# PoeBlu/open-network-insight

Hardware: AMD Instinct MI355X
Metric: netflow records scored/sec (whole node) + Gibbs iters/sec, 20-topic LDA (higher is better)
Workload: dtype fp32

## Files before the change

### csrc/kernels/corpus.hip

```cpp
#include <hipcub/hipcub.hpp>

#include "oni_common.h"

namespace {

constexpr int kB = 256;
inline unsigned nblk(int64_t n) { return (unsigned)((n + kB - 1) / kB > 0 ? (n + kB - 1) / kB : 1); }

struct Arena {
  char* base;
  size_t used = 0;
  template <class T>
  T* take(size_t n) {
    used = (used + 255) & ~size_t(255);
    T* p = base ? reinterpret_cast<T*>(base + used) : nullptr;
    used += n * sizeof(T);
    return p;
  }
};

__global__ void k_iota(int32_t* __restrict__ v, int64_t n) {
  const int64_t i = (int64_t)blockIdx.x * kB + threadIdx.x;
  if (i < n) v[i] = (int32_t)i;
}
// ... 139 lines not shown
  const int64_t i = (int64_t)blockIdx.x * kB + threadIdx.x;
  if (i >= n_chunks) return;
  int64_t lo = 0, hi = D;
  while (hi - lo > 1) {
    const int64_t mid = (lo + hi) >> 1;
    if (chunk_first[mid] <= i) lo = mid; else hi = mid;
  }
  const int64_t c = i - chunk_first[lo];
  const int64_t nt = tok_ptr[lo + 1] - tok_ptr[lo];
  const int64_t p0 = c * L;
  const int64_t ln = nt - p0 < L ? nt - p0 : L;
  cdoc[i] = (int32_t)lo;
  cpos0[i] = (int32_t)p0;
  clen[i] = (int32_t)ln;
  cmulti[i] = (chunk_first[lo + 1] - chunk_first[lo]) > 1 ? 1 : 0;
  key[i] = (uint32_t)(L - ln);
}

__global__ void k_chunk_gather(const int32_t* __restrict__ order, int64_t n_chunks, int64_t n_pad_total,
                               const int32_t* __restrict__ cdoc, const int32_t* __restrict__ cpos0,
                               const int32_t* __restrict__ clen, const uint8_t* __restrict__ cmulti,
                               const int32_t* __restrict__ doc_keys, int32_t* __restrict__ o_doc,
                               int32_t* __restrict__ o_pos0, int32_t* __restrict__ o_len, uint8_t* __restrict__ o_multi,
                               int32_t* __restrict__ o_key) {
  const int64_t i = (int64_t)blockIdx.x * kB + threadIdx.x;
  if (i >= n_pad_total) return;
  if (i < n_chunks) {
    const int32_t s = order[i];
    const int32_t d = cdoc[s];
    o_doc[i] = d;
    o_pos0[i] = cpos0[s];
    o_len[i] = clen[s];
    o_multi[i] = cmulti[s];
    o_key[i] = doc_keys[d];
  } else {
    o_doc[i] = -1;
    o_pos0[i] = 0;
    o_len[i] = 0;
    o_multi[i] = 0;
    o_key[i] = 0;
  }
}

__global__ void k_slice_len(const int32_t* __restrict__ o_len, int64_t ns, int S, int32_t* __restrict__ slice_len,
                            int64_t* __restrict__ slice_w) {
  const int64_t s = (int64_t)blockIdx.x * kB + threadIdx.x;
  if (s < ns) {
    slice_len[s] = o_len[s * S];
    slice_w[s] = (int64_t)o_len[s * S] * S;
  }
  if (s == ns) slice_w[ns] = 0;
}

__global__ void k_word_keys(const uint32_t* __restrict__ tok_word, int64_t n, uint32_t V, uint32_t* __restrict__ key) {
  const int64_t i = (int64_t)blockIdx.x * kB + threadIdx.x;
  if (i < n) {
    const uint32_t w = tok_word[i];
    key[i] = w == oni::kPadWord ? V : w;
  }
}

__global__ void k_word_index(const uint32_t* __restrict__ ks, const int32_t* __restrict__ slot, int64_t T, int tile,
                             int32_t* __restrict__ wpos, int32_t* __restrict__ tile_wlo,
                             int32_t* __restrict__ tile_whi) {
  const int64_t i = (int64_t)blockIdx.x * kB + threadIdx.x;
  if (i >= T) return;
  wpos[slot[i]] = (int32_t)i;
  if (i % tile == 0) {
    const int64_t t = i / tile;
    const int64_t e = i + tile - 1 < T - 1 ? i + tile - 1 : T - 1;
    tile_wlo[t] = (int32_t)ks[i];
    tile_whi[t] = (int32_t)ks[e];
  }
}

__global__ void k_fill_i32(int32_t* __restrict__ p, int64_t n, int32_t v) {
  const int64_t i = (int64_t)blockIdx.x * kB + threadIdx.x;
  if (i < n) p[i] = v;
}

#define ONI_TRY(x)                          \
  do {                                       \
    const hipError_t e_ = (x);               \
    if (e_ != hipSuccess) return (int)e_;    \
  } while (0)

int bits_for(uint64_t maxv) {
  int b = 1;
  while (b < 64 && (maxv >> b)) ++b;
  return b;
}

hipError_t window_pass(void* tmp, size_t& bytes, const int32_t* perm, int32_t* keys_out, const int32_t* val,
                       int32_t* val_out, int64_t n, hipStream_t s) {
  const int pbits = bits_for(n > 1 ? (uint64_t)(n - 1) : 1);
  const int lo = pbits > 8 ? pbits - 8 : 0;
  return hipcub::DeviceRadixSort::SortPairs(tmp, bytes, reinterpret_cast<const uint32_t*>(perm),
                                            reinterpret_cast<uint32_t*>(keys_out), val, val_out, (int)n, lo, pbits,
                                            s);
}

__global__ void k_scatter(const int32_t* __restrict__ dst, const int32_t* __restrict__ val, int64_t n,
                          int32_t* __restrict__ out) {
  const unsigned per = gridDim.x / 8u;
  const unsigned t = (blockIdx.x % 8u) * per + blockIdx.x / 8u;
  const int64_t i = (int64_t)t * kB + threadIdx.x;
  if (i < n) out[dst[i]] = val[i];
}

inline unsigned nblk8(int64_t n) { return (nblk(n) + 7u) & ~7u; }

}

template <class K>
static int dict_encode_impl(const uint64_t* keys, int64_t n, int key_bits, uint64_t* uniq, int32_t* ids,
                            int64_t* n_uniq, const int32_t* weight, int64_t* counts, void* tmp, size_t* tmp_bytes,
                            hipStream_t s) {
  constexpr bool kNarrow = sizeof(K) == 4;
  Arena ar{static_cast<char*>(tmp)};
  K* kin = kNarrow ? ar.take<K>(n) : nullptr;
  K* ks = ar.take<K>(n);
// ... 281 lines not shown
    return 0;
  }
  if (nnz > 0) k_doc_pair_ptr<<<nblk(nnz), kB, 0, s>>>(pair_doc, nnz, D, doc_pair_ptr);
  else k_fill_i32<<<1, kB, 0, s>>>(reinterpret_cast<int32_t*>(doc_pair_ptr), 2 * (D + 1), 0);
  k_i32_to_i64<<<nblk(nnz + 1), kB, 0, s>>>(pair_cnt, nnz, c64);
  ONI_TRY(hipcub::DeviceScan::ExclusiveSum(cub, cbytes, c64, glob, (int)(nnz + 1), s));
  k_doc_tok<<<nblk(D + 1), kB, 0, s>>>(doc_pair_ptr, glob, D, L, doc_tok_ptr, nch, is_long);
  k_pair_tokoff<<<nblk(nnz), kB, 0, s>>>(pair_doc, glob, doc_tok_ptr, nnz, pair_tokoff);
  ONI_TRY(hipcub::DeviceScan::ExclusiveSum(cub, cbytes, nch, chunk_first, (int)(D + 1), s));
  k_iota<<<nblk(D), kB, 0, s>>>(iota, D);
  if (D > 0) ONI_TRY(hipcub::DeviceSelect::Flagged(cub, cbytes, iota, is_long, long_rows, n_long, (int)D, s));
  else ONI_TRY(hipMemsetAsync(n_long, 0, sizeof(int32_t), s));
  k_scalars3<<<1, 64, 0, s>>>(glob + nnz, chunk_first + D, n_long, scalars);
  return (int)hipGetLastError();
}

ONI_API int oni_chunk_layout(const int64_t* chunk_first, const int64_t* doc_tok_ptr, const int32_t* doc_keys,
                             int64_t D, int64_t n_chunks, int L, int S, int32_t* chunk_doc, int32_t* chunk_pos0,
                             int32_t* chunk_len, uint8_t* chunk_multi, int32_t* chunk_key, int32_t* slice_len,
                             int64_t* slice_off, void* tmp, size_t* tmp_bytes, hipStream_t s) {
  const int64_t ns = (n_chunks + S - 1) / S;
  Arena ar{static_cast<char*>(tmp)};
  int32_t* cdoc = ar.take<int32_t>(n_chunks);
  int32_t* cpos0 = ar.take<int32_t>(n_chunks);
  int32_t* clen = ar.take<int32_t>(n_chunks);
  uint8_t* cmul = ar.take<uint8_t>(n_chunks);
  uint32_t* key = ar.take<uint32_t>(n_chunks);
  uint32_t* ks = ar.take<uint32_t>(n_chunks);
  int32_t* iota = ar.take<int32_t>(n_chunks);
  int32_t* order = ar.take<int32_t>(n_chunks);
  int64_t* sw = ar.take<int64_t>(ns + 1);
  const int kbits = bits_for((uint64_t)L);
  size_t b1 = 0, b2 = 0;
  ONI_TRY(hipcub::DeviceRadixSort::SortPairs(nullptr, b1, key, ks, iota, order, (int)n_chunks, 0, kbits, s));
  ONI_TRY(hipcub::DeviceScan::ExclusiveSum(nullptr, b2, sw, slice_off, (int)(ns + 1), s));
  void* cub = ar.take<char>(b1 > b2 ? b1 : b2);
  if (!tmp) {
    *tmp_bytes = ar.used + 256;
    return 0;
  }
  size_t cbytes = b1 > b2 ? b1 : b2;
  if (n_chunks > 0) {
    k_chunks<<<nblk(n_chunks), kB, 0, s>>>(chunk_first, doc_tok_ptr, D, n_chunks, L, cdoc, cpos0, clen, cmul, key);
    k_iota<<<nblk(n_chunks), kB, 0, s>>>(iota, n_chunks);
    ONI_TRY(hipcub::DeviceRadixSort::SortPairs(cub, cbytes, key, ks, iota, order, (int)n_chunks, 0, kbits, s));
  }
  k_chunk_gather<<<nblk(ns * S), kB, 0, s>>>(order, n_chunks, ns * S, cdoc, cpos0, clen, cmul, doc_keys, chunk_doc,
                                            chunk_pos0, chunk_len, chunk_multi, chunk_key);
  k_slice_len<<<nblk(ns + 1), kB, 0, s>>>(chunk_len, ns, S, slice_len, sw);
  ONI_TRY(hipcub::DeviceScan::ExclusiveSum(cub, cbytes, sw, slice_off, (int)(ns + 1), s));
  return (int)hipGetLastError();
}

ONI_API int oni_word_index(const uint32_t* tok_word, int64_t slots, int64_t T, int64_t V, int tile,
                           int32_t* wsorted, int32_t* wslot, int32_t* wpos, int32_t* tile_wlo, int32_t* tile_whi,
                           void* tmp, size_t* tmp_bytes, hipStream_t s) {
  if (slots >= (int64_t)1 << 31) return (int)hipErrorInvalidValue;
  Arena ar{static_cast<char*>(tmp)};
  uint32_t* key = ar.take<uint32_t>(slots);
  uint32_t* ks = reinterpret_cast<uint32_t*>(wsorted);
  int32_t* iota = ar.take<int32_t>(slots);
  int32_t* slot = wslot;
  const int kbits = bits_for((uint64_t)V);
  size_t b1 = 0;
  ONI_TRY(hipcub::DeviceRadixSort::SortPairs(nullptr, b1, key, ks, iota, slot, (int)slots, 0, kbits, s));
  void* cub = ar.take<char>(b1);
  if (!tmp) {
    *tmp_bytes = ar.used + 256;
    return 0;
  }
  k_fill_i32<<<nblk(slots), kB, 0, s>>>(wpos, slots, -1);
  if (slots == 0) return (int)hipGetLastError();
  k_word_keys<<<nblk(slots), kB, 0, s>>>(tok_word, slots, (uint32_t)V, key);
  k_iota<<<nblk(slots), kB, 0, s>>>(iota, slots);
  ONI_TRY(hipcub::DeviceRadixSort::SortPairs(cub, b1, key, ks, iota, slot, (int)slots, 0, kbits, s));
  if (T > 0) k_word_index<<<nblk(T), kB, 0, s>>>(ks, slot, T, tile, wpos, tile_wlo, tile_whi);
  return (int)hipGetLastError();
}
```

### csrc/kernels/glue.hip

```cpp
#include "oni_common.h"

namespace {

__global__ __launch_bounds__(256) void k_widen_pair(const uint32_t* __restrict__ a, const uint32_t* __restrict__ b,
                                                    int64_t n, uint64_t* __restrict__ out) {
  const int64_t stride = (int64_t)gridDim.x * blockDim.x;
  for (int64_t i = (int64_t)blockIdx.x * blockDim.x + threadIdx.x; i < n; i += stride) {
    out[i] = (uint64_t)a[i];
    out[n + i] = (uint64_t)b[i];
  }
}

}

ONI_API int oni_widen_pair(const uint32_t* a, const uint32_t* b, int64_t n, uint64_t* out, hipStream_t s) {
  if (n <= 0) return 0;
  k_widen_pair<<<oni::grid_for(n, 256, 8192), 256, 0, s>>>(a, b, n, out);
  return (int)hipGetLastError();
}
```

### csrc/kernels/sell.hip

```cpp
#include "oni_common.h"

namespace {

__device__ __forceinline__ int64_t find_pair(const int64_t* __restrict__ tokoff, int64_t lo, int64_t hi, int64_t pos) {
  while (hi - lo > 1) {
    const int64_t mid = (lo + hi) >> 1;
    if (tokoff[mid] <= pos) lo = mid; else hi = mid;
  }
  return lo;
}

__global__ void k_sell_fill(const int32_t* __restrict__ chunk_doc, const int32_t* __restrict__ chunk_pos0,
                            const int32_t* __restrict__ chunk_len, int64_t n_chunks, int S,
                            const int64_t* __restrict__ slice_off, const int64_t* __restrict__ doc_pair_ptr,
                            const int64_t* __restrict__ pair_tokoff, const int32_t* __restrict__ pair_word,
                            const int32_t* __restrict__ pair_cnt, uint32_t* __restrict__ tok_word) {
  const int64_t i = (int64_t)blockIdx.x * blockDim.x + threadIdx.x;
  if (i >= n_chunks) return;
  const int d = chunk_doc[i];
  if (d < 0) return;
  const int64_t slice = i / S, lane = i % S;
  const int64_t off = slice_off[slice] + lane;
  const int64_t pos0 = chunk_pos0[i];
  const int len = chunk_len[i];
  int64_t j = find_pair(pair_tokoff, doc_pair_ptr[d], doc_pair_ptr[d + 1], pos0);
  int64_t end = pair_tokoff[j] + pair_cnt[j];
  uint32_t w = (uint32_t)pair_word[j];
  for (int s = 0; s < len; ++s) {
    const int64_t pos = pos0 + s;
    while (end <= pos) {
      ++j;
      end = pair_tokoff[j] + pair_cnt[j];
      w = (uint32_t)pair_word[j];
    }
    tok_word[off + (int64_t)s * S] = w;
  }
}

__global__ void k_sell_perm_z(const int32_t* __restrict__ chunk_doc, const int32_t* __restrict__ chunk_pos0,
                              const int32_t* __restrict__ chunk_len, int64_t n_chunks, int S,
                              const int64_t* __restrict__ slice_off, const int64_t* __restrict__ doc_tok_ptr,
                              uint8_t* __restrict__ tok_z, uint8_t* __restrict__ canon_z, int dir) {
  const int64_t i = (int64_t)blockIdx.x * blockDim.x + threadIdx.x;
  if (i >= n_chunks) return;
  const int d = chunk_doc[i];
  if (d < 0) return;
  const int64_t slice = i / S, lane = i % S;
  const int64_t off = slice_off[slice] + lane;
  const int64_t base = doc_tok_ptr[d] + chunk_pos0[i];
  const int len = chunk_len[i];
  for (int s = 0; s < len; ++s) {
    if (dir == 0) canon_z[base + s] = tok_z[off + (int64_t)s * S];
    else tok_z[off + (int64_t)s * S] = canon_z[base + s];
  }
}

}

ONI_API int oni_sell_fill(const int32_t* chunk_doc, const int32_t* chunk_pos0, const int32_t* chunk_len,
                          int64_t n_chunks, int S, const int64_t* slice_off, const int64_t* doc_pair_ptr,
                          const int64_t* pair_tokoff, const int32_t* pair_word, const int32_t* pair_cnt,
                          uint32_t* tok_word, hipStream_t s) {
  const unsigned grid = (unsigned)((n_chunks + 255) / 256);
  if (grid == 0) return 0;
  k_sell_fill<<<grid, 256, 0, s>>>(chunk_doc, chunk_pos0, chunk_len, n_chunks, S, slice_off, doc_pair_ptr,
                                   pair_tokoff, pair_word, pair_cnt, tok_word);
  return (int)hipGetLastError();
}

ONI_API int oni_sell_perm_z(const int32_t* chunk_doc, const int32_t* chunk_pos0, const int32_t* chunk_len,
                            int64_t n_chunks, int S, const int64_t* slice_off, const int64_t* doc_tok_ptr,
                            uint8_t* tok_z, uint8_t* canon_z, int dir, hipStream_t s) {
  const unsigned grid = (unsigned)((n_chunks + 255) / 256);
  if (grid == 0) return 0;
  k_sell_perm_z<<<grid, 256, 0, s>>>(chunk_doc, chunk_pos0, chunk_len, n_chunks, S, slice_off, doc_tok_ptr, tok_z,
                                     canon_z, dir);
  return (int)hipGetLastError();
}
```

### oni355/ops/__init__.py

```python
from __future__ import annotations

import os

import ctypes as C
import enum
from typing import NamedTuple

import numpy as np
import torch

from ..ref import spec
from . import _lib

__all__ = [
    "f32_keys", "i64_keys", "quantile_cuts", "bin_keys", "flow_keys", "flow_wordify", "sell_fill",
    "sell_perm_z", "gibbs_pass", "foldin_pass", "prior_rows", "theta_rows_prior", "table_lookup", "gibbs_which", "GibbsKernel", "gibbs_apply", "mh_tables", "SAMPLER_MH", "CountMode", "copy_rows", "score", "select_below", "choose_tiling",
]


def _is_dev(t: torch.Tensor) -> bool:
    return t.device.type == "cuda"


def _u32np(t: torch.Tensor) -> np.ndarray:
# ... 520 lines not shown
              wsum: torch.Tensor | None = None, wcdf: torch.Tensor | None = None) -> None:
    cdf = wcdf is not None
    if cdf == (walias is not None) or (walias is not None and wsum is None):
        raise ValueError("one word proposal table: walias + wsum, or wcdf")
    if cdf and (wcdf.shape != (q.shape[0], spec.MH_CDF_BUCKETS) or wcdf.dtype != torch.float32):
        raise ValueError("wcdf must be a [V, 16] float32 table")
    if not _is_dev(q):
        wt, ws, da, gg = spec.mh_tables(q.numpy(), nk.numpy(), ndk_src.numpy(), long_rows.numpy(), K, alpha, vbeta,
                                        word="cdf" if cdf else "alias")
        if cdf:
            wcdf.copy_(torch.from_numpy(wt))
        else:
            walias.copy_(torch.from_numpy(wt.view(np.int32)))
            wsum.copy_(torch.from_numpy(ws))
        if da.shape[0]:
            dalias.copy_(torch.from_numpy(da.view(np.int32)))
        g.copy_(torch.from_numpy(gg))
        return
    V, KS = q.shape
    p = lambda t: _lib.ptr(t) if t is not None else None
    _lib.check(_lib.lib().oni_mh_tables(_lib.ptr(q), V, K, KS, _lib.ptr(ndk_src), _lib.ptr(long_rows),
                                        long_rows.numel(), float(alpha), p(walias), p(wsum), p(wcdf),
                                        _lib.ptr(dalias), _lib.ptr(nk), float(vbeta), _lib.ptr(g), _lib.stream()),
               "oni_mh_tables")


def delta_recount(wslot, tile_wlo, tile_whi, chg_mask, tok_word, tok_z, tok_zprev, dnwk_out, KS: int, G: int) -> None:
    T = wslot.numel()
    if T == 0:
        return
    if not _is_dev(tok_z):
        sl = wslot.long()
        zn, zo = tok_z[sl].long(), tok_zprev[sl].long()
        ch = zn != zo
        w = tok_word[sl][ch].long()
        one = torch.ones(int(ch.sum()), dtype=torch.int32)
        dnwk_out.view(-1).index_add_(0, w * KS + zn[ch], one)
        dnwk_out.view(-1).index_add_(0, w * KS + zo[ch], -one)
        tok_zprev[sl[ch]] = tok_z[sl[ch]]
        return
    S = 64 // G
    wmax = max(1, RECOUNT_CELLS // KS)
    _lib.check(_lib.lib().oni_delta_recount(*map(_lib.ptr, (wslot, tile_wlo, tile_whi, chg_mask, tok_word, tok_z,
                                                            tok_zprev)), T, _lib.ptr(dnwk_out), KS,
                                            S.bit_length() - 1, G, RECOUNT_TILE, wmax, _lib.stream()),
               "oni_delta_recount")


WBITS_BLOCK = 8192


def wdelta_records(wsorted: torch.Tensor) -> torch.Tensor:
    T = wsorted.numel()
    out = torch.zeros((max(T, 1), 2), dtype=torch.int16, device=wsorted.device)
    if T:
        nb = -(-T // WBITS_BLOCK)
        w = torch.nn.functional.pad(wsorted.to(torch.int32), (0, nb * WBITS_BLOCK - T)).view(nb, WBITS_BLOCK)
        rel = (w - w[:, :1]).view(-1)[:T].clamp_(max=0xFFFF)
        out[:T, 1] = torch.where(rel >= 0x8000, rel - 0x10000, rel).to(torch.int16)
    return out.view(torch.int32).view(-1)


def wdelta_recount(wbits, wsorted, zz_w, dnwk_out, KS: int) -> None:
    T = wsorted.numel()
    if T == 0:
        return
    if not _is_dev(wsorted):
        b = wbits.numpy().view(np.uint32)
        pos = np.nonzero(np.unpackbits(b.view(np.uint8), bitorder="little")[:T])[0]
        pt = torch.from_numpy(pos)
        w = wsorted[pt].long()
        one = torch.ones(pos.size, dtype=torch.int32)
        zz = zz_w[pt].to(torch.int64) & 0xFFFF
        dnwk_out.view(-1).index_add_(0, w * KS + (zz >> 8), one)
        dnwk_out.view(-1).index_add_(0, w * KS + (zz & 0xFF), -one)
        wbits.zero_()
        return
    if zz_w.dtype != torch.int32 or zz_w.numel() < T:
        raise ValueError("zz_w must be the int32 [T] record array of wdelta_records")
    wmax = max(1, RECOUNT_CELLS // KS)
    _lib.check(_lib.lib().oni_wdelta_recount(*map(_lib.ptr, (wbits, wsorted, zz_w)), T, _lib.ptr(dnwk_out), KS,
                                             wmax, _lib.stream()), "oni_wdelta_recount")


RECOUNT_TILE = 4096
DN_AUX = 4
RECOUNT_CELLS = 2048


def exact_guard(ndk: torch.Tensor, rows: torch.Tensor, K: int, limit: int, flag: torch.Tensor) -> None:
    KS = ndk.shape[-1]
    if not _is_dev(ndk):
        ok = not bool((ndk[rows.long(), :K] > limit).any()) if rows.numel() else True
        flag.fill_(1 if ok else 0)
        return
    _lib.check(_lib.lib().oni_exact_guard(_lib.ptr(ndk), _lib.ptr(rows), int(rows.numel()), KS, K, int(limit),
                                          _lib.ptr(flag), _lib.stream()), "oni_exact_guard")


def recount(wsorted, wslot, tok_z, nwk_out, KS: int) -> None:
    T = wsorted.numel()
    if T == 0:
        return
    if not _is_dev(tok_z):
        z = (tok_z[wslot.long()] if wslot is not None else tok_z[:T]).long()
        nwk_out.view(-1).index_add_(0, wsorted.long() * KS + z, torch.ones_like(z, dtype=torch.int32))
# ... 333 lines not shown
```

### oni355/ops/_lib.py

```python
from __future__ import annotations

import ctypes as C
import os
import threading

import torch

_HERE = os.path.dirname(os.path.abspath(__file__))
LIB_DIR = os.path.join(os.path.dirname(_HERE), "_lib")
HIP_LIB_PATH = os.path.join(LIB_DIR, "liboni_hip.so")

_lock = threading.Lock()
_lib = None

vp, i32, i64, f32, u32 = C.c_void_p, C.c_int32, C.c_int64, C.c_float, C.c_uint32


class OniGibbs(C.Structure):

    _fields_ = [
        ("tok_word", vp), ("tok_z", vp), ("slice_off", vp), ("slice_len", vp),
        ("chunk_doc", vp), ("chunk_pos0", vp), ("chunk_key", vp), ("chunk_multi", vp),
        ("ndk_src", vp), ("ndk_dst", vp), ("q", vp), ("qfix", vp), ("dnwk", vp), ("dnk", vp), ("sweep_ctr", vp), ("chg_mask", vp),
        ("wpos", vp), ("z_w", vp), ("zz_w", vp), ("chg_count", vp), ("exact_guard", vp), ("tok_zlag", vp),
        ("n_slices", i64), ("K", i32), ("KS", i32), ("alpha", f32), ("seed0", u32), ("seed1", u32),
        ("nk_rep", i32), ("flags", i32),
    ]


class OniMH(C.Structure):

    _fields_ = [
        ("g", OniGibbs), ("walias", vp), ("wsum", vp), ("wcdf", vp), ("dalias", vp), ("mh_g", vp), ("chunk_dslot", vp),
        ("chunk_len", vp), ("kalpha", f32), ("inv_alpha", f32), ("lmax", i32), ("doc_moves", i32), ("wp", i32),
    ]


class OniFoldin(C.Structure):

    _fields_ = [
        ("tok_word", vp), ("tok_z", vp), ("slice_off", vp), ("slice_len", vp),
        ("chunk_doc", vp), ("chunk_pos0", vp), ("chunk_key", vp), ("chunk_multi", vp),
        ("ndk_src", vp), ("ndk_dst", vp), ("phi", vp), ("ndk_sum", vp),
        ("n_slices", i64), ("K", i32), ("KS", i32), ("alpha", f32), ("seed0", u32), ("seed1", u32),
        ("sweep_lo", i32), ("n_sweeps", i32), ("avg_from", i32), ("select", i32),
        ("prior", vp),
    ]


_REGISTRY: dict[str, list] = {
    "oni_radix_hist": [vp, i64, C.c_int, C.c_int, vp, C.c_int, u32, vp, vp],
    "oni_f32_keys": [vp, i64, vp, vp],
    "oni_i64_keys": [vp, i64, vp, vp],
    "oni_bin_keys": [vp, i64, vp, C.c_int, vp, vp],
    "oni_flow_keys": [vp, vp, vp, vp, vp, i64, vp, vp, vp, vp],
    "oni_flow_wordify": [vp, vp, vp, vp, vp, i64, vp, C.c_int, C.c_int, C.c_int, vp, vp, vp],
    "oni_sell_fill": [vp, vp, vp, i64, C.c_int, vp, vp, vp, vp, vp, vp, vp],
    "oni_sell_perm_z": [vp, vp, vp, i64, C.c_int, vp, vp, vp, vp, C.c_int, vp],
    "oni_gibbs_launch": [C.POINTER(OniGibbs), C.c_int, C.c_int, C.c_int, C.c_int, C.c_int, vp],
    "oni_gibbs_which": [C.POINTER(OniGibbs), C.c_int, C.c_int, C.c_int, C.c_int, C.c_int, C.POINTER(C.c_int),
                        C.POINTER(C.c_int)],
    "oni_gibbs_sizeof_args": [],
    "oni_exact_guard": [vp, vp, i64, C.c_int, C.c_int, C.c_int32, vp, vp],
    "oni_gibbs_mh_launch": [C.POINTER(OniMH), C.c_int, C.c_int, vp],
    "oni_mh_sizeof_args": [],
    "oni_mh_tables": [vp, i64, C.c_int, C.c_int, vp, vp, i64, f32, vp, vp, vp, vp, vp, f32, vp, vp],
    "oni_widen_pair": [vp, vp, i64, vp, vp],
    "oni_quantile_pick": [vp, vp, C.c_int, C.c_int, C.c_int, vp, vp, vp],
    "oni_tail_grid": [],
    "oni_tail_sums": [vp, vp, vp, vp, i64, i64, C.c_int, C.c_int, C.c_double, C.c_double, C.c_double, C.c_double,
                      vp, vp, vp],
    "oni_theta_rows": [vp, i64, C.c_int, C.c_int, f32, f32, vp, C.c_int, vp],
    "oni_theta_rows_prior": [vp, vp, i64, C.c_int, C.c_int, f32, vp, C.c_int, vp],
    "oni_prior_rows": [vp, vp, vp, i64, vp, i64, C.c_int, C.c_int, f32, f32, vp, vp],
    "oni_phi_rows": [vp, vp, i64, C.c_int, C.c_int, f32, f32, vp, C.c_int, C.c_int, vp],
    "oni_gibbs_apply": [vp, vp, vp, vp, vp, vp, vp, i64, C.c_int, C.c_int, f32, f32, vp, C.c_int, C.c_int, C.c_int,
                        vp, vp, vp, i64, vp, vp, vp, C.c_int, vp, i64, C.c_int, vp],
    "oni_recount": [vp, vp, vp, i64, vp, C.c_int, C.c_int, C.c_int, vp],
    "oni_recount_stream": [vp, vp, i64, vp, C.c_int, C.c_int, C.c_int, vp],
    "oni_delta_recount": [vp, vp, vp, vp, vp, vp, vp, i64, vp, C.c_int, C.c_int, C.c_int, C.c_int, C.c_int, vp],
    "oni_copy_rows": [vp, vp, vp, i64, C.c_int, vp],
    "oni_x01_pack": [vp, vp, i64, vp, i64, vp, i64, C.c_int, i64, i64, C.c_int, C.c_int, vp, vp],
    "oni_x01_unpack": [vp, vp, i64, vp, i64, vp, i64, C.c_int, i64, i64, C.c_int, C.c_int, vp, vp],
    "oni_score": [vp, vp, C.c_int, vp, vp, vp, vp, i64, f32, vp, vp, vp, vp, vp],
    "oni_select_below": [vp, i64, f32, u32, vp, vp, vp, i64, vp],
    "oni_pair_score": [vp, vp, C.c_int, vp, vp, i64, vp, vp],
    "oni_event_min": [vp, vp, vp, i64, f32, vp, vp, vp, vp, vp],
    "oni_tile_score": [vp, vp, C.c_int, vp, vp, vp, vp, i64, vp, vp],
    "oni_wdelta_recount": [vp, vp, vp, i64, vp, C.c_int, C.c_int, vp],
    "oni_foldin_launch": [C.POINTER(OniFoldin), C.c_int, C.c_int, C.c_int, vp],
    "oni_foldin_sizeof_args": [],
    "oni_table_lookup": [vp, vp, i64, vp, i64, vp, vp, vp],
}
_ARG_STRUCTS = {"oni_gibbs_sizeof_args": OniGibbs, "oni_mh_sizeof_args": OniMH, "oni_foldin_sizeof_args": OniFoldin}


def _bind(h: C.CDLL, name: str, argtypes: list) -> None:
    try:
        fn = getattr(h, name)
    except AttributeError:
        raise RuntimeError(f"{HIP_LIB_PATH} has no symbol {name}: stale or broken build, "
                           "rebuild with `python tools/build.py`") from None
    fn.argtypes = argtypes
    fn.restype = C.c_int


def register(name: str, argtypes: list) -> None:
    with _lock:
        _REGISTRY[name] = argtypes
        if _lib is not None:
            _bind(_lib, name, argtypes)


def lib() -> C.CDLL:
    global _lib
    if _lib is not None:
        return _lib
    with _lock:
        if _lib is not None:
            return _lib
# ... 36 lines not shown
```

### oni355/ops/corpus.py

```python
from __future__ import annotations

import ctypes as C
from dataclasses import dataclass

import torch

from . import _lib

vp, i64, ci = C.c_void_p, C.c_int64, C.c_int
_SZ = C.POINTER(C.c_size_t)
_lib.register("oni_dict_encode", [vp, i64, ci, vp, vp, vp, vp, vp, vp, _SZ, vp])
_lib.register("oni_hashdict_build", [vp, i64, i64, vp, vp, vp, vp, vp])
_lib.register("oni_hashdict_finish", [vp, i64, ci, i64, vp, vp, vp, i64, vp, vp, vp, _SZ, vp])
_lib.register("oni_route_pack", [vp, vp, vp, vp, vp, i64, ci, vp, vp, vp, vp, _SZ, vp])
_lib.register("oni_route_pack_ids", [vp, vp, vp, vp, vp, i64, ci, vp, vp, vp, vp, _SZ, vp])
_lib.register("oni_route_unpack", [vp, i64, ci, vp, vp, ci, vp, vp, vp, vp, vp])
_lib.register("oni_partition", [vp, vp, vp, i64, ci, vp, vp, vp, vp, vp, _SZ, vp])
_lib.register("oni_place_stats", [vp, vp, i64, vp, i64, ci, vp, vp])
_lib.register("oni_place_owner", [vp, i64, vp, i64, vp, ci, vp, vp, vp])
_lib.register("oni_pair_build", [vp, vp, vp, i64, i64, i64, vp, vp, vp, vp, vp, vp, i64, vp, _SZ, vp])
_lib.register("oni_doc_pair_build", [vp, i64, vp, ci, vp, vp, i64, i64, vp, vp, vp, vp, vp, vp, vp, vp, i64, vp, _SZ, vp])
_lib.register("oni_doc_layout", [vp, vp, i64, i64, ci, vp, vp, vp, vp, vp, vp, vp, _SZ, vp])
_lib.register("oni_chunk_layout", [vp, vp, vp, i64, i64, ci, ci, vp, vp, vp, vp, vp, vp, vp, vp, _SZ, vp])
_lib.register("oni_word_index", [vp, i64, i64, i64, ci, vp, vp, vp, vp, vp, vp, _SZ, vp])


def _call(name: str, *args) -> None:
    L = _lib.lib()
    fn = getattr(L, name)
    nb = C.c_size_t(0)
    _lib.check(fn(*args, None, C.byref(nb), _lib.stream()), name + " (size)")
    tmp = torch.empty(max(int(nb.value), 1), dtype=torch.uint8, device="cuda")
    _lib.check(fn(*args, tmp.data_ptr(), C.byref(nb), _lib.stream()), name)


def _p(t):
    return _lib.ptr(t)


HASH_DICT = True


def bits_for(maxv: int) -> int:
    return max(int(maxv).bit_length(), 1)


HASH_DICT_MIN_KEYS = 1 << 20
HASH_DICT_SLOTS = 1 << 22


def dict_encode_hash(keys64: torch.Tensor, key_bits: int, table_slots: int = HASH_DICT_SLOTS):
    n = keys64.numel()
    dev = keys64.device
    M = int(table_slots)
    tab = torch.empty(M, dtype=torch.int64, device=dev)
    val = torch.empty(M, dtype=torch.int32, device=dev)
    uns = torch.empty(M // 2 + 1, dtype=torch.int64, device=dev)
    status = torch.zeros(3, dtype=torch.int32, device=dev)
    _lib.check(_lib.lib().oni_hashdict_build(_p(keys64), n, M, _p(tab), _p(val), _p(uns), _p(status), _lib.stream()),
               "oni_hashdict_build")
    nu, ovf, _ = (int(x) for x in status.tolist())
    if ovf or nu > M // 2:
        return None
    uniq = torch.empty(max(nu, 1), dtype=torch.int64, device=dev)
    ids = torch.empty(n, dtype=torch.int32, device=dev)
    _call("oni_hashdict_finish", _p(keys64), n, int(min(max(key_bits, 1), 64)), M, _p(tab), _p(val), _p(uns), nu,
          _p(uniq), _p(ids))
    return uniq[:nu], ids


def dict_encode(keys64: torch.Tensor, key_bits: int = 64, weights: torch.Tensor | None = None,
                counts: bool = False, hashed: bool = False):
    if keys64.dtype != torch.int64 or not keys64.is_contiguous():
        raise TypeError("dict_encode: contiguous int64 keys")
    n = keys64.numel()
    if hashed and not counts and n >= HASH_DICT_MIN_KEYS and key_bits <= 62 and HASH_DICT:
        r = dict_encode_hash(keys64, key_bits)
# ... 166 lines not shown
          _p(pd), _p(pw), _p(pc), _p(tp), _p(nnz), _p(o0) if o0 is not None else None, int(n0))
    m = int(nnz.item())
    return PairSet(pd[:m], pw[:m], pc[:m], tp[:n], o0.to(torch.int64) if o0 is not None else None, int(D), int(V))


def _doc_pair_build_torch(keys64: torch.Tensor, word: torch.Tensor, V: int, weight: torch.Tensor | None, n0: int):
    from ..pipeline.common import torch_pairs
    n = keys64.numel()
    udoc, inv = torch.unique(keys64, return_inverse=True)
    tp = torch_pairs(inv.to(torch.int32), word, V)
    w = weight.to(torch.int64) if weight is not None else torch.ones(n, dtype=torch.int64, device=keys64.device)
    cnt = torch.zeros(tp.pair_doc.numel(), dtype=torch.int64, device=keys64.device).index_add_(0, tp.tok_pair.long(), w)
    o0 = torch.argsort(tp.tok_pair[:n0], stable=True) if n0 > 0 else None
    return udoc, PairSet(tp.pair_doc, tp.pair_word, cnt.clamp_(max=0x7FFFFFFF).to(torch.int32), tp.tok_pair, o0,
                         int(udoc.numel()), int(V))


def doc_pair_build(doc_keys, word: torch.Tensor, V: int, weight: torch.Tensor | None = None, n0: int = 0):
    parts = list(doc_keys) if isinstance(doc_keys, (tuple, list)) else [doc_keys]
    if not 1 <= len(parts) <= 2 or any(p.dtype != parts[0].dtype or p.device != word.device for p in parts):
        raise TypeError("doc_pair_build: doc keys are one tensor or two of one dtype, on the words' device")
    if parts[0].dtype not in (torch.int32, torch.int64) or (len(parts) == 2 and parts[0].dtype != torch.int32):
        raise TypeError("doc_pair_build: int64 keys, int32 u32 bits, or two int32 halves")
    n = word.numel()
    if word.dtype != torch.int32 or not word.is_contiguous() or sum(p.numel() for p in parts) != n:
        raise TypeError(f"doc_pair_build: word must be contiguous int32, one per doc key [{n}]")
    if weight is not None and (weight.dtype != torch.int32 or weight.numel() != n):
        raise TypeError("doc_pair_build: weight must be int32 [n]")
    if not 0 <= n0 <= n:
        raise ValueError("doc_pair_build: n0 out of range")
    if V < 1:
        raise ValueError("doc_pair_build: V >= 1")
    dev = word.device
    if dev.type != "cuda":
        k = torch.cat(parts) if len(parts) == 2 else parts[0]
        return _doc_pair_build_torch(k.to(torch.int64) & 0xFFFFFFFF, word, V, weight, n0)
    parts = [p.contiguous() for p in parts]
    uniq = torch.empty(max(n, 1), dtype=torch.int64, device=dev)
    nu = torch.zeros(2, dtype=torch.int64, device=dev)
    pd = torch.empty(max(n, 1), dtype=torch.int32, device=dev)
    pw = torch.empty_like(pd)
    pc = torch.empty_like(pd)
    tp = torch.empty_like(pd)
    o0 = torch.empty(n0, dtype=torch.int32, device=dev) if n0 > 0 else None
    _call("oni_doc_pair_build", _p(parts[0]) if parts[0].numel() else None, parts[0].numel(),
          _p(parts[1]) if len(parts) == 2 and parts[1].numel() else None, parts[0].element_size(), _p(word) if n else None,
          _p(weight.contiguous()) if weight is not None else None, n, int(V), _p(uniq), _lib.ptr(nu), _p(pd), _p(pw),
          _p(pc), _p(tp), _lib.ptr(nu) + 8, _p(o0) if o0 is not None else None, int(n0))
    D, m = (int(x) for x in nu.tolist())
    return uniq[:D], PairSet(pd[:m], pw[:m], pc[:m], tp[:n], o0.to(torch.int64) if o0 is not None else None, D, int(V))


def corpus_layout(ps: PairSet, doc_keys: torch.Tensor, G: int, L: int, recount_tile: int):
    from .. import ops
    dev = ps.pair_doc.device
    D, V, nnz = ps.D, ps.V, ps.nnz
    S = 64 // G
    i64t, i32t = torch.int64, torch.int32
    doc_pair_ptr = torch.empty(D + 1, dtype=i64t, device=dev)
    doc_tok_ptr = torch.empty(D + 1, dtype=i64t, device=dev)
    pair_tokoff = torch.empty(max(nnz, 1), dtype=i64t, device=dev)
    chunk_first = torch.empty(D + 1, dtype=i64t, device=dev)
    long_rows = torch.empty(max(D, 1), dtype=i32t, device=dev)
    scal = torch.zeros(3, dtype=i64t, device=dev)
    _call("oni_doc_layout", _p(ps.pair_doc) if nnz else None, _p(ps.pair_cnt) if nnz else None, nnz, D, int(L),
          _p(doc_pair_ptr), _p(doc_tok_ptr), _p(pair_tokoff), _p(chunk_first), _p(long_rows), _p(scal))
    T, n_chunks, n_long = (int(x) for x in scal.tolist())
    ns = (n_chunks + S - 1) // S
    dk = doc_keys.to(i32t).contiguous()
    chunk_doc = torch.empty(max(ns * S, 1), dtype=i32t, device=dev)
    chunk_pos0 = torch.empty_like(chunk_doc)
    chunk_len = torch.empty_like(chunk_doc)
    chunk_multi = torch.empty(max(ns * S, 1), dtype=torch.uint8, device=dev)
    chunk_key = torch.empty_like(chunk_doc)
    slice_len = torch.empty(max(ns, 1), dtype=i32t, device=dev)
    slice_off = torch.empty(ns + 1, dtype=i64t, device=dev)
    _call("oni_chunk_layout", _p(chunk_first), _p(doc_tok_ptr), _p(dk) if D else None, D, n_chunks, int(L), S,
          _p(chunk_doc), _p(chunk_pos0), _p(chunk_len), _p(chunk_multi), _p(chunk_key), _p(slice_len),
          _p(slice_off))
    total = int(slice_off[-1].item())
    chunk_doc, chunk_pos0, chunk_len = chunk_doc[: ns * S], chunk_pos0[: ns * S], chunk_len[: ns * S]
    chunk_multi, chunk_key, slice_len = chunk_multi[: ns * S], chunk_key[: ns * S], slice_len[:ns]
    tok_word = torch.full((max(total, 1),), -1, dtype=i32t, device=dev)
    if n_chunks:
        ops.sell_fill(chunk_doc, chunk_pos0, chunk_len, S, slice_off[:ns].contiguous(), doc_pair_ptr,
                      pair_tokoff[:nnz].contiguous(), ps.pair_word, ps.pair_cnt, tok_word)
    slots = tok_word.numel()
    n_tiles = (T + recount_tile - 1) // recount_tile
    wsorted = torch.empty(max(slots, 1), dtype=i32t, device=dev)
    wslot = torch.empty_like(wsorted)
    wpos = torch.empty(slots, dtype=i32t, device=dev)
    tile_wlo = torch.empty(max(n_tiles, 1), dtype=i32t, device=dev)
    tile_whi = torch.empty_like(tile_wlo)
    _call("oni_word_index", _p(tok_word), slots, T, V, int(recount_tile), _p(wsorted), _p(wslot), _p(wpos),
          _p(tile_wlo), _p(tile_whi))
    return dict(T=T, doc_pair_ptr=doc_pair_ptr, doc_tok_ptr=doc_tok_ptr, pair_tokoff=pair_tokoff[:nnz],
                slice_off=slice_off[:ns].contiguous(), slice_len=slice_len, chunk_doc=chunk_doc,
                chunk_pos0=chunk_pos0, chunk_len=chunk_len, chunk_key=chunk_key, chunk_multi=chunk_multi,
                tok_word=tok_word, long_rows=long_rows[:n_long], wsorted=wsorted[:T], wslot=wslot[:T],
                tile_wlo=tile_wlo[:n_tiles], tile_whi=tile_whi[:n_tiles], wpos=wpos)
```

Before: 230.7 million.

## Fuse SELL fill with sort-key/iota generation and add device wdelta_records kernel

The SELL fill kernel now also writes pad words and the slot iota, so the word index sort reads tok_word directly as keys. This removes the separate full-tensor init, key-mapping, iota and wpos fill kernels. wpos is now written for every slot by the index kernel. A new device kernel replaces the torch-based wdelta_records path. This trims launches and passes in corpus setup, but it depends on the pad word sorting above all valid words within kbits and changes the record format to packed int32.

```diff
diff --git a/csrc/kernels/corpus.hip b/csrc/kernels/corpus.hip
--- a/csrc/kernels/corpus.hip
+++ b/csrc/kernels/corpus.hip
@@ -215,21 +215,13 @@
   if (s == ns) slice_w[ns] = 0;
 }
 
-__global__ void k_word_keys(const uint32_t* __restrict__ tok_word, int64_t n, uint32_t V, uint32_t* __restrict__ key) {
-  const int64_t i = (int64_t)blockIdx.x * kB + threadIdx.x;
-  if (i < n) {
-    const uint32_t w = tok_word[i];
-    key[i] = w == oni::kPadWord ? V : w;
-  }
-}
-
-__global__ void k_word_index(const uint32_t* __restrict__ ks, const int32_t* __restrict__ slot, int64_t T, int tile,
-                             int32_t* __restrict__ wpos, int32_t* __restrict__ tile_wlo,
+__global__ void k_word_index(const uint32_t* __restrict__ ks, const int32_t* __restrict__ slot, int64_t slots,
+                             int64_t T, int tile, int32_t* __restrict__ wpos, int32_t* __restrict__ tile_wlo,
                              int32_t* __restrict__ tile_whi) {
   const int64_t i = (int64_t)blockIdx.x * kB + threadIdx.x;
-  if (i >= T) return;
-  wpos[slot[i]] = (int32_t)i;
-  if (i % tile == 0) {
+  if (i >= slots) return;
+  wpos[slot[i]] = i < T ? (int32_t)i : -1;
+  if (i < T && i % tile == 0) {
     const int64_t t = i / tile;
     const int64_t e = i + tile - 1 < T - 1 ? i + tile - 1 : T - 1;
     tile_wlo[t] = (int32_t)ks[i];
@@ -617,28 +609,23 @@
   return (int)hipGetLastError();
 }
 
-ONI_API int oni_word_index(const uint32_t* tok_word, int64_t slots, int64_t T, int64_t V, int tile,
-                           int32_t* wsorted, int32_t* wslot, int32_t* wpos, int32_t* tile_wlo, int32_t* tile_whi,
-                           void* tmp, size_t* tmp_bytes, hipStream_t s) {
-  if (slots >= (int64_t)1 << 31) return (int)hipErrorInvalidValue;
+ONI_API int oni_word_index(const uint32_t* tok_word, const int32_t* slot_iota, int64_t slots, int64_t T, int64_t V,
+                           int tile, int32_t* wsorted, int32_t* wslot, int32_t* wpos, int32_t* tile_wlo,
+                           int32_t* tile_whi, void* tmp, size_t* tmp_bytes, hipStream_t s) {
+  if (slots < 0 || slots >= (int64_t)1 << 31 || T < 0 || T > slots || V < 1 || V >= (int64_t)1 << 31 || tile < 1)
+    return (int)hipErrorInvalidValue;
   Arena ar{static_cast<char*>(tmp)};
-  uint32_t* key = ar.take<uint32_t>(slots);
   uint32_t* ks = reinterpret_cast<uint32_t*>(wsorted);
-  int32_t* iota = ar.take<int32_t>(slots);
-  int32_t* slot = wslot;
   const int kbits = bits_for((uint64_t)V);
   size_t b1 = 0;
-  ONI_TRY(hipcub::DeviceRadixSort::SortPairs(nullptr, b1, key, ks, iota, slot, (int)slots, 0, kbits, s));
+  ONI_TRY(hipcub::DeviceRadixSort::SortPairs(nullptr, b1, tok_word, ks, slot_iota, wslot, (int)slots, 0, kbits, s));
   void* cub = ar.take<char>(b1);
   if (!tmp) {
     *tmp_bytes = ar.used + 256;
     return 0;
   }
-  k_fill_i32<<<nblk(slots), kB, 0, s>>>(wpos, slots, -1);
-  if (slots == 0) return (int)hipGetLastError();
-  k_word_keys<<<nblk(slots), kB, 0, s>>>(tok_word, slots, (uint32_t)V, key);
-  k_iota<<<nblk(slots), kB, 0, s>>>(iota, slots);
-  ONI_TRY(hipcub::DeviceRadixSort::SortPairs(cub, b1, key, ks, iota, slot, (int)slots, 0, kbits, s));
-  if (T > 0) k_word_index<<<nblk(T), kB, 0, s>>>(ks, slot, T, tile, wpos, tile_wlo, tile_whi);
+  if (slots == 0) return 0;
+  ONI_TRY(hipcub::DeviceRadixSort::SortPairs(cub, b1, tok_word, ks, slot_iota, wslot, (int)slots, 0, kbits, s));
+  k_word_index<<<nblk(slots), kB, 0, s>>>(ks, wslot, slots, T, tile, wpos, tile_wlo, tile_whi);
   return (int)hipGetLastError();
 }
diff --git a/csrc/kernels/glue.hip b/csrc/kernels/glue.hip
--- a/csrc/kernels/glue.hip
+++ b/csrc/kernels/glue.hip
@@ -11,6 +11,22 @@
   }
 }
 
+__global__ __launch_bounds__(256) void k_wdelta_records(const int32_t* __restrict__ wsorted, int64_t T, int block,
+                                                        uint32_t* __restrict__ rec) {
+  const int64_t stride = (int64_t)gridDim.x * blockDim.x;
+  for (int64_t i = (int64_t)blockIdx.x * blockDim.x + threadIdx.x; i < T; i += stride) {
+    const int32_t rel = wsorted[i] - wsorted[i - i % block];
+    rec[i] = (uint32_t)(rel < 0xFFFF ? rel : 0xFFFF) << 16;
+  }
+}
+
+}
+
+ONI_API int oni_wdelta_records(const int32_t* wsorted, int64_t T, int block, uint32_t* rec, hipStream_t s) {
+  if (T < 0 || block < 1) return (int)hipErrorInvalidValue;
+  if (T == 0) return 0;
+  k_wdelta_records<<<oni::grid_for(T, 256, 8192), 256, 0, s>>>(wsorted, T, block, rec);
+  return (int)hipGetLastError();
 }
 
 ONI_API int oni_widen_pair(const uint32_t* a, const uint32_t* b, int64_t n, uint64_t* out, hipStream_t s) {
diff --git a/csrc/kernels/sell.hip b/csrc/kernels/sell.hip
--- a/csrc/kernels/sell.hip
+++ b/csrc/kernels/sell.hip
@@ -10,30 +10,52 @@
   return lo;
 }
 
+template <bool FULL>
 __global__ void k_sell_fill(const int32_t* __restrict__ chunk_doc, const int32_t* __restrict__ chunk_pos0,
                             const int32_t* __restrict__ chunk_len, int64_t n_chunks, int S,
                             const int64_t* __restrict__ slice_off, const int64_t* __restrict__ doc_pair_ptr,
                             const int64_t* __restrict__ pair_tokoff, const int32_t* __restrict__ pair_word,
-                            const int32_t* __restrict__ pair_cnt, uint32_t* __restrict__ tok_word) {
+                            const int32_t* __restrict__ pair_cnt, uint32_t* __restrict__ tok_word,
+                            int32_t* __restrict__ slot_iota) {
   const int64_t i = (int64_t)blockIdx.x * blockDim.x + threadIdx.x;
   if (i >= n_chunks) return;
   const int d = chunk_doc[i];
-  if (d < 0) return;
+  if (!FULL && d < 0) return;
   const int64_t slice = i / S, lane = i % S;
   const int64_t off = slice_off[slice] + lane;
-  const int64_t pos0 = chunk_pos0[i];
-  const int len = chunk_len[i];
-  int64_t j = find_pair(pair_tokoff, doc_pair_ptr[d], doc_pair_ptr[d + 1], pos0);
-  int64_t end = pair_tokoff[j] + pair_cnt[j];
-  uint32_t w = (uint32_t)pair_word[j];
-  for (int s = 0; s < len; ++s) {
-    const int64_t pos = pos0 + s;
-    while (end <= pos) {
-      ++j;
-      end = pair_tokoff[j] + pair_cnt[j];
-      w = (uint32_t)pair_word[j];
+  const int len = d < 0 ? 0 : chunk_len[i];
+  if (d >= 0) {
+    const int64_t pos0 = chunk_pos0[i];
+    int64_t j = find_pair(pair_tokoff, doc_pair_ptr[d], doc_pair_ptr[d + 1], pos0);
+    int64_t end = pair_tokoff[j] + pair_cnt[j];
+    uint32_t w = (uint32_t)pair_word[j];
+    for (int s = 0; s < len; ++s) {
+      const int64_t pos = pos0 + s;
+      while (end <= pos) {
+        ++j;
+        end = pair_tokoff[j] + pair_cnt[j];
+        w = (uint32_t)pair_word[j];
+      }
+      const int64_t o = off + (int64_t)s * S;
+      tok_word[o] = w;
+      if constexpr (FULL) slot_iota[o] = (int32_t)o;
     }
-    tok_word[off + (int64_t)s * S] = w;
+  }
+  if constexpr (FULL) {
+    const int slen = chunk_len[slice * S];
+    for (int s = len; s < slen; ++s) {
+      const int64_t o = off + (int64_t)s * S;
+      tok_word[o] = oni::kPadWord;
+      slot_iota[o] = (int32_t)o;
+    }
+  }
+}
+
+__global__ void k_sell_pad(uint32_t* __restrict__ tok_word, int32_t* __restrict__ slot_iota, int64_t slots) {
+  const int64_t i = (int64_t)blockIdx.x * blockDim.x + threadIdx.x;
+  if (i < slots) {
+    tok_word[i] = oni::kPadWord;
+    slot_iota[i] = (int32_t)i;
   }
 }
 
@@ -63,8 +85,24 @@
                           uint32_t* tok_word, hipStream_t s) {
   const unsigned grid = (unsigned)((n_chunks + 255) / 256);
   if (grid == 0) return 0;
-  k_sell_fill<<<grid, 256, 0, s>>>(chunk_doc, chunk_pos0, chunk_len, n_chunks, S, slice_off, doc_pair_ptr,
-                                   pair_tokoff, pair_word, pair_cnt, tok_word);
+  k_sell_fill<false><<<grid, 256, 0, s>>>(chunk_doc, chunk_pos0, chunk_len, n_chunks, S, slice_off, doc_pair_ptr,
+                                          pair_tokoff, pair_word, pair_cnt, tok_word, nullptr);
+  return (int)hipGetLastError();
+}
+
+ONI_API int oni_sell_fill_index(const int32_t* chunk_doc, const int32_t* chunk_pos0, const int32_t* chunk_len,
+                                int64_t n_chunks, int S, const int64_t* slice_off, const int64_t* doc_pair_ptr,
+                                const int64_t* pair_tokoff, const int32_t* pair_word, const int32_t* pair_cnt,
+                                uint32_t* tok_word, int32_t* slot_iota, int64_t slots, hipStream_t s) {
+  if (slots < 0 || slots >= (int64_t)1 << 31 || n_chunks < 0 || S < 1 || n_chunks % S != 0)
+    return (int)hipErrorInvalidValue;
+  if (n_chunks == 0) {
+    if (slots > 0) k_sell_pad<<<(unsigned)((slots + 255) / 256), 256, 0, s>>>(tok_word, slot_iota, slots);
+    return (int)hipGetLastError();
+  }
+  k_sell_fill<true><<<(unsigned)((n_chunks + 255) / 256), 256, 0, s>>>(
+      chunk_doc, chunk_pos0, chunk_len, n_chunks, S, slice_off, doc_pair_ptr, pair_tokoff, pair_word, pair_cnt,
+      tok_word, slot_iota);
   return (int)hipGetLastError();
 }
 
diff --git a/oni355/ops/__init__.py b/oni355/ops/__init__.py
--- a/oni355/ops/__init__.py
+++ b/oni355/ops/__init__.py
@@ -596,6 +596,14 @@
 
 def wdelta_records(wsorted: torch.Tensor) -> torch.Tensor:
     T = wsorted.numel()
+    if _is_dev(wsorted):
+        if T == 0:
+            return torch.zeros(1, dtype=torch.int32, device=wsorted.device)
+        _need(wsorted, torch.int32, "wsorted")
+        rec = torch.empty(T, dtype=torch.int32, device=wsorted.device)
+        _lib.check(_lib.lib().oni_wdelta_records(_lib.ptr(wsorted), T, WBITS_BLOCK, _lib.ptr(rec), _lib.stream()),
+                   "oni_wdelta_records")
+        return rec
     out = torch.zeros((max(T, 1), 2), dtype=torch.int16, device=wsorted.device)
     if T:
         nb = -(-T // WBITS_BLOCK)
diff --git a/oni355/ops/_lib.py b/oni355/ops/_lib.py
--- a/oni355/ops/_lib.py
+++ b/oni355/ops/_lib.py
@@ -66,6 +66,7 @@
     "oni_mh_sizeof_args": [],
     "oni_mh_tables": [vp, i64, C.c_int, C.c_int, vp, vp, i64, f32, vp, vp, vp, vp, vp, f32, vp, vp],
     "oni_widen_pair": [vp, vp, i64, vp, vp],
+    "oni_wdelta_records": [vp, i64, C.c_int, vp, vp],
     "oni_quantile_pick": [vp, vp, C.c_int, C.c_int, C.c_int, vp, vp, vp],
     "oni_tail_grid": [],
     "oni_tail_sums": [vp, vp, vp, vp, i64, i64, C.c_int, C.c_int, C.c_double, C.c_double, C.c_double, C.c_double,
diff --git a/oni355/ops/corpus.py b/oni355/ops/corpus.py
--- a/oni355/ops/corpus.py
+++ b/oni355/ops/corpus.py
@@ -22,7 +22,8 @@
 _lib.register("oni_doc_pair_build", [vp, i64, vp, ci, vp, vp, i64, i64, vp, vp, vp, vp, vp, vp, vp, vp, i64, vp, _SZ, vp])
 _lib.register("oni_doc_layout", [vp, vp, i64, i64, ci, vp, vp, vp, vp, vp, vp, vp, _SZ, vp])
 _lib.register("oni_chunk_layout", [vp, vp, vp, i64, i64, ci, ci, vp, vp, vp, vp, vp, vp, vp, vp, _SZ, vp])
-_lib.register("oni_word_index", [vp, i64, i64, i64, ci, vp, vp, vp, vp, vp, vp, _SZ, vp])
+_lib.register("oni_sell_fill_index", [vp, vp, vp, i64, ci, vp, vp, vp, vp, vp, vp, vp, i64, vp])
+_lib.register("oni_word_index", [vp, vp, i64, i64, i64, ci, vp, vp, vp, vp, vp, vp, _SZ, vp])
 
 
 def _call(name: str, *args) -> None:
@@ -295,7 +296,6 @@
 
 
 def corpus_layout(ps: PairSet, doc_keys: torch.Tensor, G: int, L: int, recount_tile: int):
-    from .. import ops
     dev = ps.pair_doc.device
     D, V, nnz = ps.D, ps.V, ps.nnz
     S = 64 // G
@@ -324,19 +324,21 @@
     total = int(slice_off[-1].item())
     chunk_doc, chunk_pos0, chunk_len = chunk_doc[: ns * S], chunk_pos0[: ns * S], chunk_len[: ns * S]
     chunk_multi, chunk_key, slice_len = chunk_multi[: ns * S], chunk_key[: ns * S], slice_len[:ns]
-    tok_word = torch.full((max(total, 1),), -1, dtype=i32t, device=dev)
-    if n_chunks:
-        ops.sell_fill(chunk_doc, chunk_pos0, chunk_len, S, slice_off[:ns].contiguous(), doc_pair_ptr,
-                      pair_tokoff[:nnz].contiguous(), ps.pair_word, ps.pair_cnt, tok_word)
-    slots = tok_word.numel()
+    slots = max(total, 1)
+    tok_word = torch.empty(slots, dtype=i32t, device=dev)
+    slot_iota = torch.empty(slots, dtype=i32t, device=dev)
+    _lib.check(_lib.lib().oni_sell_fill_index(
+        _p(chunk_doc), _p(chunk_pos0), _p(chunk_len), ns * S, S, _p(slice_off), _p(doc_pair_ptr), _p(pair_tokoff),
+        _p(ps.pair_word) if nnz else None, _p(ps.pair_cnt) if nnz else None, _p(tok_word), _p(slot_iota), slots,
+        _lib.stream()), "oni_sell_fill_index")
     n_tiles = (T + recount_tile - 1) // recount_tile
-    wsorted = torch.empty(max(slots, 1), dtype=i32t, device=dev)
+    wsorted = torch.empty(slots, dtype=i32t, device=dev)
     wslot = torch.empty_like(wsorted)
     wpos = torch.empty(slots, dtype=i32t, device=dev)
     tile_wlo = torch.empty(max(n_tiles, 1), dtype=i32t, device=dev)
     tile_whi = torch.empty_like(tile_wlo)
-    _call("oni_word_index", _p(tok_word), slots, T, V, int(recount_tile), _p(wsorted), _p(wslot), _p(wpos),
-          _p(tile_wlo), _p(tile_whi))
+    _call("oni_word_index", _p(tok_word), _p(slot_iota), slots, T, V, int(recount_tile), _p(wsorted), _p(wslot),
+          _p(wpos), _p(tile_wlo), _p(tile_whi))
     return dict(T=T, doc_pair_ptr=doc_pair_ptr, doc_tok_ptr=doc_tok_ptr, pair_tokoff=pair_tokoff[:nnz],
                 slice_off=slice_off[:ns].contiguous(), slice_len=slice_len, chunk_doc=chunk_doc,
                 chunk_pos0=chunk_pos0, chunk_len=chunk_len, chunk_key=chunk_key, chunk_multi=chunk_multi,
```

Result: no change. 231.9 million, median of 6 (+0.5%).
